# bluenote-1577/skani

Measured on NVIDIA H100. Metric: genome-pairs/sec, skani triangle 5k x 5 Mbp synthetic, higher is better.
Workload: dtype u64

## Files before the change

skani_b200/csrc/chain.cu:

```cuda
#include <cub/cub.cuh>

#include <algorithm>
#include <cmath>
#include <cstdlib>
#include <cstring>
#include <limits>
#include <numeric>

#include "chain_core.cuh"
#include "sk_internal.h"

namespace sk {

namespace tables {
#include "gbdt_tables.inc"
}

__constant__ unsigned char c_gbdt_feat[2][1365];
__constant__ float c_gbdt_thr[2][1365];
__constant__ float c_gbdt_leaf[2][1560];
__constant__ float c_gbdt_shrink[2];
__constant__ float c_gbdt_bias[2];

struct SetView {
// ... 1195 lines not shown
    feat[0][i] = tables::SK_GBDT_C125_FEAT[i]; feat[1][i] = tables::SK_GBDT_C200_FEAT[i];
    thr[0][i] = b2f(tables::SK_GBDT_C125_THR[i]); thr[1][i] = b2f(tables::SK_GBDT_C200_THR[i]);
  }
  for (int i = 0; i < 1560; i++) { leaf[0][i] = b2f(tables::SK_GBDT_C125_LEAF[i]); leaf[1][i] = b2f(tables::SK_GBDT_C200_LEAF[i]); }
  shrink[0] = b2f(SK_GBDT_C125_SHRINK_BITS); shrink[1] = b2f(SK_GBDT_C200_SHRINK_BITS);
  bias[0] = b2f(SK_GBDT_C125_BIAS_BITS); bias[1] = b2f(SK_GBDT_C200_BIAS_BITS);
  SK_CUDA(cudaMemcpyToSymbol(c_gbdt_feat, feat, sizeof(feat)));
  SK_CUDA(cudaMemcpyToSymbol(c_gbdt_thr, thr, sizeof(thr)));
  SK_CUDA(cudaMemcpyToSymbol(c_gbdt_leaf, leaf, sizeof(leaf)));
  SK_CUDA(cudaMemcpyToSymbol(c_gbdt_shrink, shrink, sizeof(shrink)));
  SK_CUDA(cudaMemcpyToSymbol(c_gbdt_bias, bias, sizeof(bias)));
  SK_CUDA(cudaDeviceSynchronize());
  if (ctx->device < 64) g_tables_uploaded[ctx->device] = true;
  return SK_OK;
}

static SetView view_of(const sk_sketch_set* s) {
  SetView v;
  v.pv_kmer = s->pv_kmer; v.pv_pos = s->pv_pos; v.pv_cc = s->pv_cc; v.pv_mult = s->pv_mult;
  v.kv_pos = s->kv_pos; v.kv_cc = s->kv_cc; v.ukmer = s->ukmer; v.ustart = s->ustart; v.ctg_rec_off = s->ctg_rec_off; v.ubucket = s->ubucket; v.htab = s->htab;
  return v;
}

static void build_meta(const sk_sketch_set* s, std::vector<GenomeMeta>& out) {
  out.resize(s->G);
  std::vector<uint32_t> tmp;
  for (uint32_t g = 0; g < s->G; g++) {
    GenomeMeta& m = out[g];
    m.seed_off = s->seed_off[g]; m.uk_off = s->uk_off[g]; m.ctg_off = s->ctg_off[g];
    m.n_rec = (uint32_t)(s->seed_off[g + 1] - s->seed_off[g]);
    m.n_uk = (uint32_t)(s->uk_off[g + 1] - s->uk_off[g]);
    m.n_ctg = (uint32_t)(s->ctg_off[g + 1] - s->ctg_off[g]);
    m.g = g; m.total_len = s->total_len[g]; m.pad = 0;
    m.ht_off = s->ht_off.empty() ? 0 : s->ht_off[g];
    m.ht_cap = s->ht_off.empty() ? 0 : (uint32_t)(s->ht_off[g + 1] - s->ht_off[g]);
    tmp.assign(s->ctg_len.begin() + s->ctg_off[g], s->ctg_len.begin() + s->ctg_off[g + 1]);
    uint64_t max_chunks = 0;
    for (uint32_t len : tmp) max_chunks += (len + (uint64_t)FRAGMENT_LENGTH - 1) / FRAGMENT_LENGTH;
    m.max_chunks = (uint32_t)std::min<uint64_t>(max_chunks, 0xFFFFFFFFu);
    std::sort(tmp.begin(), tmp.end());
    size_t n = tmp.size();
    m.q10 = n ? tmp[n * 10 / 100] : 0; m.q50 = n ? tmp[n * 50 / 100] : 0; m.q90 = n ? tmp[n * 90 / 100] : 0;
  }
}

static bool pair_switched(const sk_sketch_set* refs, uint32_t r, const sk_sketch_set* qs, uint32_t q, bool same_set) {
  auto mean_len = [](const sk_sketch_set* s, uint32_t g) {
    double sum = 0;
    for (uint64_t c = s->ctg_off[g]; c < s->ctg_off[g + 1]; c++) sum += (double)s->ctg_len[c];
    return sum / (double)(s->ctg_off[g + 1] - s->ctg_off[g]);
  };
  double mean_q = mean_len(qs, q), mean_r = mean_len(refs, r);
  double qp, rp;
  if (qs->total_len[q] > 100000 && refs->total_len[r] > 100000) {
    qp = (double)(qs->mk_off[q + 1] - qs->mk_off[q]) * (double)qs->sp.c;
    rp = (double)(refs->mk_off[r + 1] - refs->mk_off[r]) * (double)refs->sp.c;
  } else {
    qp = (double)qs->total_len[q]; rp = (double)refs->total_len[r];
  }
  double score_query = qp * std::min(mean_q, 300000.);
  double score_ref = rp * std::min(mean_r, 300000.);
  if (score_query == score_ref) {
    uint64_t rq = qs->name_rank[q] + ((same_set || qs->ranks_user_set) ? 0 : refs->G), rr = refs->name_rank[r];
    return rq > rr;
  }
  return score_query > score_ref;
}

struct BatchBuffers {
  std::vector<std::pair<void**, size_t>> reg;
};

template <typename T>
static int ensure(sk_ctx* ctx, T** p, size_t* cap, size_t need) {
  if (need <= *cap && *p) return SK_OK;
  if (*p) SK_CUDA(cudaFree(*p));
  *p = nullptr;
  size_t n = std::max<size_t>(need + need / 4, 1024);
  SK_CUDA(cudaMalloc((void**)p, n * sizeof(T)));
  *cap = n;
  return SK_OK;
}

struct ChainScratch {
  Workspace ws{};
  size_t cap_rec = 0, cap_pair = 0, cap_anc = 0, cap_chunk = 0, cap_iv = 0;
  size_t c_rec_nh = 0, c_rec_rs = 0, c_tile_off = 0;
  size_t c_stg_first = 0, c_stg_qctg = 0, c_stg_lo = 0, c_stg_hi = 0;
  size_t c_pairA = 0, c_pairC = 0, c_pairAbase = 0, c_pairCbase = 0, c_pairIbase = 0, c_pair_nint = 0, c_pair_sumlen = 0,
         c_pair_nchains = 0, c_pair_tqb = 0;
  size_t c_anc = 0, c_score = 0, c_ptr = 0, c_rootkey = 0, c_depth = 0;
  size_t c_chunk_size = 0, c_chunk_size_sorted = 0, c_chunk_id = 0, c_chunk_perm = 0, c_sort_tmp = 0;
  uint8_t* sort_tmp = nullptr;
  uint32_t* dbg_counts = nullptr; size_t c_dbg_counts = 0;
  size_t c_chunk_first = 0, c_chunk_pair = 0, c_chunk_qctg = 0, c_chunk_lo = 0, c_chunk_hi = 0, c_acc_total = 0, c_acc_rq0 = 0,
         c_acc_rq1 = 0, c_acc_tbcq = 0, c_acc_nint = 0, c_chunk_head = 0, c_chunk_est = 0, c_chunk_w = 0, c_chunk_valid = 0, c_chunk_nseeds = 0;
  size_t c_iv = 0, c_iv_keys = 0, c_iv_order = 0, c_iv_kept = 0, c_iv_next = 0, c_acc_list = 0, c_est_sorted = 0, c_w_sorted = 0;
  PairDesc* d_pairs = nullptr; size_t c_pairs = 0;
  sk_ani_result* d_out = nullptr; size_t c_out = 0;
  GenomeMeta *d_m0 = nullptr, *d_m1 = nullptr;
  size_t c_m0 = 0, c_m1 = 0;
  void free_all() {
    void* ptrs[] = {ws.chunk_size, ws.chunk_size_sorted, ws.chunk_id, ws.chunk_perm, sort_tmp, dbg_counts, ws.rec_nh, ws.rec_rs, ws.tile_off, ws.stg_first, ws.stg_qctg, ws.stg_lo, ws.stg_hi,
                    ws.pairA, ws.pairC, ws.pairAbase, ws.pairCbase, ws.pairIbase, ws.pair_nint, ws.pair_sumlen, ws.pair_nchains, ws.pair_tqb_ns, ws.anc,
                    ws.score, ws.ptr, ws.rootkey, ws.depth, ws.chunk_first, ws.chunk_pair, ws.chunk_qctg, ws.chunk_lo, ws.chunk_hi,
                    ws.acc_total, ws.acc_rq0, ws.acc_rq1, ws.acc_tbcq, ws.acc_nint, ws.chunk_head, ws.chunk_est, ws.chunk_w, ws.chunk_valid,
                    ws.chunk_nseeds, ws.iv, ws.iv_keys, ws.iv_order, ws.iv_kept, ws.iv_next, ws.acc_list, ws.est_sorted, ws.w_sorted, d_pairs, d_out, d_m0, d_m1};
    for (void* p : ptrs) if (p) cudaFree(p);
  }
};

struct HostPair { uint32_t ref, query; };

template <bool TAPS, int GL, int NE>
static int launch_dp_group(sk_ctx* ctx, uint32_t grid, uint64_t TC, const ChainParams& prm, const Workspace& ws, int dp_minb) {
  cudaStream_t st = ctx->stream;
  if (prm.band == GL * NE && dp_minb > 1) SK_LAUNCH(ctx, "dp_kernel", (dp_group_kernel<TAPS, GL, NE, true, 25><<<grid, 32, 0, st>>>(TC, prm, ws)));
  else if (prm.band == GL * NE) SK_LAUNCH(ctx, "dp_kernel", (dp_group_kernel<TAPS, GL, NE, true, 1><<<grid, 32, 0, st>>>(TC, prm, ws)));
  else SK_LAUNCH(ctx, "dp_kernel", (dp_group_kernel<TAPS, GL, NE, false, 1><<<grid, 32, 0, st>>>(TC, prm, ws)));
  return SK_OK;
}

static int launch_dp_select(sk_ctx* ctx, ChainScratch& S, uint32_t B, uint64_t TC, const ChainParams& prm, bool dp, bool taps) {
  cudaStream_t st = ctx->stream;
  Workspace& ws = S.ws;
  if (dp) {
    const uint32_t grid = (uint32_t)TC;
    const uint32_t nb = prm.band / 32 + 2;
#define DP_LAUNCH(NBV)                                                                                       \
  if (taps) SK_LAUNCH(ctx, "dp_kernel", (dp_warp_kernel<NBV, true><<<grid, 32, 0, st>>>(TC, prm, ws)));       \
  else SK_LAUNCH(ctx, "dp_kernel", (dp_warp_kernel<NBV, false><<<grid, 32, 0, st>>>(TC, prm, ws)));
    if (prm.band <= 24 && getenv("SK_DP_WARP") == nullptr) {
      const int dp_gl = getenv("SK_DP_GL") ? atoi(getenv("SK_DP_GL")) : 4;
      const int dp_minb = getenv("SK_DP_MINB") ? atoi(getenv("SK_DP_MINB")) : 25;
      const uint32_t gw = dp_gl == 4 ? 8 : 4;
      const uint32_t g4 = (uint32_t)((TC + gw - 1) / gw);
      SK_TRY(ensure(ctx, &ws.chunk_size, &S.c_chunk_size, TC)); SK_TRY(ensure(ctx, &ws.chunk_size_sorted, &S.c_chunk_size_sorted, TC));
      SK_TRY(ensure(ctx, &ws.chunk_id, &S.c_chunk_id, TC)); SK_TRY(ensure(ctx, &ws.chunk_perm, &S.c_chunk_perm, TC));
      chunk_size_kernel<<<(uint32_t)((TC + 255) / 256), 256, 0, st>>>(TC, ws); count_launch(ctx);
      size_t tb = 0;
      SK_CUDA(cub::DeviceRadixSort::SortPairsDescending(nullptr, tb, ws.chunk_size, ws.chunk_size_sorted, ws.chunk_id, ws.chunk_perm, (int)TC, 0, 32, st));
      SK_TRY(ensure(ctx, &S.sort_tmp, &S.c_sort_tmp, tb));
      SK_CUDA(cub::DeviceRadixSort::SortPairsDescending(S.sort_tmp, tb, ws.chunk_size, ws.chunk_size_sorted, ws.chunk_id, ws.chunk_perm, (int)TC, 0, 32, st));
#define DPG(GLV, NEV)                                                                                                   \
  {                                                                                                                    \
    if (taps) SK_TRY((launch_dp_group<true, GLV, NEV>(ctx, g4, TC, prm, ws, dp_minb)));                                \
    else SK_TRY((launch_dp_group<false, GLV, NEV>(ctx, g4, TC, prm, ws, dp_minb)));                                   \
  }
      if (dp_gl == 4) { if (prm.band <= 20) DPG(4, 5) else DPG(4, 6) }
      else { DPG(8, 3) }
#undef DPG
    } else if (nb <= 2) { DP_LAUNCH(2) } else if (nb <= 4) { DP_LAUNCH(4) } else if (nb <= 8) { DP_LAUNCH(8) }
    else if (nb <= 16) { DP_LAUNCH(16) } else { ctx->err = "c too small: chain band > 479 anchors is not supported"; return SK_ERR_PARAM; }
#undef DP_LAUNCH
  }
  SK_LAUNCH(ctx, "select_kernel", (select_kernel<<<B, CT, 0, st>>>(S.d_pairs, prm, ws)));
  return SK_OK;
}

static int copy_out_debug(sk_ctx* ctx, const Workspace& ws, const std::vector<PairDesc>& descs, size_t b0, uint32_t B,
                          const std::vector<uint64_t>& abase, const std::vector<uint64_t>& cbase, const std::vector<uint64_t>& ibase,
                          const uint32_t* dbg_counts, const sk_ani_result* host_out, sk_chain_debug* dbg) {
  const uint64_t TA = abase[B], TC = cbase[B], TI = ibase[B];
  std::vector<AnchorRec> anc(TA);
  std::vector<int32_t> score(TA);
  std::vector<uint32_t> ptr(TA), cq(TC), nseeds(TC), nint(B), w(TC), order(4 * TI);
  std::vector<uint64_t> cf(TC + 1);
  std::vector<IntervalKey> iv(TI);
  std::vector<uint8_t> kept(TI), valid(TC);
  std::vector<double> est(TC);
  std::vector<uint32_t> a_total(TC), a_rq0(TC), a_rq1(TC), a_tbcq(TC), a_nint(TC), counts(3 * TC);
  if (TA) {
    SK_CUDA(cudaMemcpy(anc.data(), ws.anc, TA * sizeof(AnchorRec), cudaMemcpyDeviceToHost));
    SK_CUDA(cudaMemcpy(score.data(), ws.score, TA * 4, cudaMemcpyDeviceToHost));
    SK_CUDA(cudaMemcpy(ptr.data(), ws.ptr, TA * 4, cudaMemcpyDeviceToHost));
  }
  if (TC) {
    SK_CUDA(cudaMemcpy(cf.data(), ws.chunk_first, (TC + 1) * 8, cudaMemcpyDeviceToHost));
    SK_CUDA(cudaMemcpy(cq.data(), ws.chunk_qctg, TC * 4, cudaMemcpyDeviceToHost));
    SK_CUDA(cudaMemcpy(nseeds.data(), ws.chunk_nseeds, TC * 4, cudaMemcpyDeviceToHost));
    SK_CUDA(cudaMemcpy(est.data(), ws.chunk_est, TC * 8, cudaMemcpyDeviceToHost));
    SK_CUDA(cudaMemcpy(w.data(), ws.chunk_w, TC * 4, cudaMemcpyDeviceToHost));
    SK_CUDA(cudaMemcpy(valid.data(), ws.chunk_valid, TC, cudaMemcpyDeviceToHost));
    SK_CUDA(cudaMemcpy(a_total.data(), ws.acc_total, TC * 4, cudaMemcpyDeviceToHost));
    SK_CUDA(cudaMemcpy(a_rq0.data(), ws.acc_rq0, TC * 4, cudaMemcpyDeviceToHost));
    SK_CUDA(cudaMemcpy(a_rq1.data(), ws.acc_rq1, TC * 4, cudaMemcpyDeviceToHost));
    SK_CUDA(cudaMemcpy(a_tbcq.data(), ws.acc_tbcq, TC * 4, cudaMemcpyDeviceToHost));
    SK_CUDA(cudaMemcpy(a_nint.data(), ws.acc_nint, TC * 4, cudaMemcpyDeviceToHost));
    SK_CUDA(cudaMemcpy(counts.data(), dbg_counts, TC * 12, cudaMemcpyDeviceToHost));
  }
  SK_CUDA(cudaMemcpy(nint.data(), ws.pair_nint, B * 4, cudaMemcpyDeviceToHost));
  if (TI) {
    SK_CUDA(cudaMemcpy(iv.data(), ws.iv, TI * sizeof(IntervalKey), cudaMemcpyDeviceToHost));
    SK_CUDA(cudaMemcpy(order.data(), ws.iv_order, 4 * TI * 4, cudaMemcpyDeviceToHost));
    SK_CUDA(cudaMemcpy(kept.data(), ws.iv_kept, TI, cudaMemcpyDeviceToHost));
  }
  for (uint32_t i = 0; i < B; i++) {
    sk_chain_debug* d = dbg + b0 + i;
    memset(d, 0, sizeof(*d));
    d->result = host_out[b0 + i];
    d->switched = descs[b0 + i].switched;
    const uint64_t a0 = abase[i], na = abase[i + 1] - a0, c0 = cbase[i], nc = cbase[i + 1] - c0, ib = ibase[i];
    const uint32_t ni = nint[i];
    if (ni > ibase[i + 1] - ib) { ctx->err = "chain debug: a pair has more intervals than its capacity"; return SK_ERR_STATE; }
    d->n_anchors = na; d->n_chunks = nc; d->n_intervals = ni;
    d->anchors = (uint32_t*)calloc(std::max<uint64_t>(na, 1), 20);
    d->score = (int64_t*)calloc(std::max<uint64_t>(na, 1), 8);
    d->pointer = (uint32_t*)calloc(std::max<uint64_t>(na, 1), 4);
    d->chunk_first = (uint32_t*)calloc(nc + 1, 4);
    d->chunk_nseeds = (uint32_t*)calloc(std::max<uint64_t>(nc, 1), 4);
    d->intervals = (int64_t*)calloc(std::max<uint32_t>(ni, 1), 11 * 8);
    d->chunk_stats = (uint32_t*)calloc(std::max<uint64_t>(nc, 1), 9 * 4);
    if (!d->anchors || !d->score || !d->pointer || !d->chunk_first || !d->chunk_nseeds || !d->intervals || !d->chunk_stats) {
      ctx->err = "chain debug: out of host memory"; return SK_ERR_STATE;
    }
    for (uint64_t c = 0; c < nc; c++) {
      const uint64_t x0 = cf[c0 + c] - a0, x1 = cf[c0 + c + 1] - a0;
      if (x0 > x1 || x1 > na) { ctx->err = "chain debug: chunk outside its pair's anchors"; return SK_ERR_STATE; }
      d->chunk_first[c] = (uint32_t)x0; d->chunk_nseeds[c] = nseeds[c0 + c];
      const uint64_t g = c0 + c;
      const uint32_t st[9] = {a_total[g], a_rq0[g], a_rq1[g], a_tbcq[g], a_nint[g], nseeds[g], counts[3 * g], counts[3 * g + 1],
                              counts[3 * g + 2]};
      memcpy(d->chunk_stats + 9 * c, st, sizeof(st));
      for (uint64_t x = x0; x < x1; x++) {
        const AnchorRec& a = anc[a0 + x];
        uint32_t* o = d->anchors + 5 * x;
        o[0] = cq[c0 + c]; o[1] = a.qpos; o[2] = a.rc >> 1; o[3] = a.rpos; o[4] = a.rc & 1u;
        d->score[x] = score[a0 + x]; d->pointer[x] = ptr[a0 + x];
      }
    }
    d->chunk_first[nc] = (uint32_t)na;
    uint32_t npow2 = 1;
    while (npow2 < ni) npow2 <<= 1;
    for (uint32_t j = 0; j < ni; j++) {
      const uint32_t oj = order[4 * ib + npow2 + j];
      if (oj >= ni) { ctx->err = "chain debug: interval order out of range"; return SK_ERR_STATE; }
      const IntervalKey& x = iv[ib + oj];
      int64_t* o = d->intervals + 11 * j;
      o[0] = iv_score(x); o[1] = iv_num_anchors(x); o[2] = iv_q0(x); o[3] = iv_q1(x); o[4] = iv_r0(x); o[5] = iv_r1(x);
      o[6] = iv_rctg(x); o[7] = iv_qctg(x); o[8] = iv_chunk(x); o[9] = iv_rev(x); o[10] = kept[ib + oj];
    }
    std::vector<std::pair<double, uint64_t>> es;
    for (uint64_t c = c0; c < c0 + nc; c++) if (valid[c]) es.push_back({est[c], w[c]});
    std::sort(es.begin(), es.end());
    d->n_ests = es.size();
    d->est = (double*)calloc(std::max<size_t>(es.size(), 1), 8);
    d->weight = (uint64_t*)calloc(std::max<size_t>(es.size(), 1), 8);
    if (!d->est || !d->weight) { ctx->err = "chain debug: out of host memory"; return SK_ERR_STATE; }
    for (size_t j = 0; j < es.size(); j++) { d->est[j] = es[j].first; d->weight[j] = es[j].second; }
  }
  return SK_OK;
}

static int run_batch(sk_ctx* ctx, ChainScratch& S, const sk_sketch_set* refs, const sk_sketch_set* qs, const std::vector<PairDesc>& descs,
                     size_t b0, size_t b1, uint64_t total_rec, uint64_t total_chunks, const std::vector<uint32_t>& tile_off, const ChainParams& prm, const SetView& v0, const SetView& v1,
                     sk_ani_result* host_out, sk_chain_debug* dbg) {
  cudaStream_t st = ctx->stream;
  const uint32_t B = (uint32_t)(b1 - b0);
  Workspace& ws = S.ws;
  const size_t NR = std::max<uint64_t>(total_rec, 1);
#define ENS(field, capf, n) SK_TRY(ensure(ctx, &ws.field, &S.capf, n))
  const size_t NS = std::max<uint64_t>(total_chunks, 1);
  ENS(rec_nh, c_rec_nh, NR); ENS(rec_rs, c_rec_rs, NR); ENS(tile_off, c_tile_off, B + 1);
  ENS(stg_first, c_stg_first, NS); ENS(stg_qctg, c_stg_qctg, NS); ENS(stg_lo, c_stg_lo, NS); ENS(stg_hi, c_stg_hi, NS);
  ENS(pairA, c_pairA, B); ENS(pairC, c_pairC, B); ENS(pairAbase, c_pairAbase, B + 1); ENS(pairCbase, c_pairCbase, B + 1);
  ENS(pairIbase, c_pairIbase, B + 1); ENS(pair_nint, c_pair_nint, B); ENS(pair_sumlen, c_pair_sumlen, B); ENS(pair_nchains, c_pair_nchains, B);
  ENS(pair_tqb_ns, c_pair_tqb, B);
  SK_TRY(ensure(ctx, &S.d_pairs, &S.c_pairs, B));
  SK_TRY(ensure(ctx, &S.d_out, &S.c_out, B));
  SK_CUDA(h2d_small(ctx, S.d_pairs, descs.data() + b0, B * sizeof(PairDesc)));
  SK_CUDA(cudaMemsetAsync(ws.pair_nint, 0, B * 4, st));
  SK_CUDA(cudaMemsetAsync(ws.pair_sumlen, 0, B * 4, st));
  SK_CUDA(cudaMemsetAsync(ws.pair_nchains, 0, B * 4, st));
  SK_CUDA(cudaMemsetAsync(ws.pair_tqb_ns, 0, B * 4, st));
  SK_CUDA(cudaMemsetAsync(ws.pairA, 0, B * 4, st));
  SK_CUDA(h2d_small(ctx, ws.tile_off, tile_off.data(), (B + 1) * 4));

  const uint32_t n_tiles = tile_off[B];
  if (n_tiles > 0) {
    size_t n_small = 0;
    for (size_t i = b0; i < b1; i++) {
      const PairDesc& d = descs[i];
      if (!d.valid) continue;
      const sk_sketch_set* rs_ = d.rset ? qs : refs;
      if (!rs_->ht_off.empty()) { const uint64_t cap = rs_->ht_off[d.rg + 1] - rs_->ht_off[d.rg]; if (cap && cap <= PROBE_STAGE_ENTRIES) n_small++; }
    }
    const bool staged = (getenv("SK_PROBE_TMA") ? atoi(getenv("SK_PROBE_TMA")) != 0 : true) && 2 * n_small >= (size_t)B;
    if (staged) SK_LAUNCH(ctx, "probe_kernel", (probe_kernel<true, PROBE_MINB><<<n_tiles, CT, 0, st>>>(S.d_pairs, B, v0, v1, S.d_m0, S.d_m1, prm, ws)));
    else SK_LAUNCH(ctx, "probe_kernel", (probe_kernel<false, PROBE_MINB><<<n_tiles, CT, 0, st>>>(S.d_pairs, B, v0, v1, S.d_m0, S.d_m1, prm, ws)));
  }
  std::vector<uint32_t> hA(B), hC(B);
  SK_CUDA(cudaMemcpyAsync(hA.data(), ws.pairA, B * 4, cudaMemcpyDeviceToHost, st));
  SK_CUDA(cudaStreamSynchronize(st));
  SK_CUDA(cudaGetLastError());
  std::vector<uint64_t> abase(B + 1, 0), cbase(B + 1, 0), ibase(B + 1, 0);
  for (uint32_t i = 0; i < B; i++) {
    abase[i + 1] = abase[i] + hA[i];
    ibase[i + 1] = ibase[i] + hA[i] / 3;
  }
  const uint64_t TA = abase[B], TI = ibase[B];
  SK_CUDA(h2d_small(ctx, ws.pairAbase, abase.data(), (B + 1) * 8));
  SK_CUDA(h2d_small(ctx, ws.pairIbase, ibase.data(), (B + 1) * 8));
  const size_t NA = std::max<uint64_t>(TA, 1), NI = std::max<uint64_t>(TI, 1);
  ENS(anc, c_anc, NA);
  SK_CUDA(cudaFuncSetAttribute(chunk_anchor_kernel<CHUNK_ANCHOR_MINB>, cudaFuncAttributeMaxDynamicSharedMemorySize,
                               (int)sizeof(ChunkAnchorSmem)));
  SK_LAUNCH(ctx, "chunk_anchor_kernel", (chunk_anchor_kernel<CHUNK_ANCHOR_MINB><<<B, CT, sizeof(ChunkAnchorSmem), st>>>(S.d_pairs, v0, v1, S.d_m0, S.d_m1, ws)));
  SK_CUDA(cudaMemcpyAsync(hC.data(), ws.pairC, B * 4, cudaMemcpyDeviceToHost, st));
  SK_CUDA(cudaStreamSynchronize(st));
  SK_CUDA(cudaGetLastError());
  for (uint32_t i = 0; i < B; i++) {
    if (hC[i] > descs[b0 + i].max_chunks) { ctx->err = "chain: a pair has more chunks than its contig-length bound"; return SK_ERR_STATE; }
    cbase[i + 1] = cbase[i] + hC[i];
  }
  const uint64_t TC = cbase[B];
  SK_CUDA(h2d_small(ctx, ws.pairCbase, cbase.data(), (B + 1) * 8));
  const size_t NCH = std::max<uint64_t>(TC, 1);
  ENS(score, c_score, dbg ? NA : 1); ENS(ptr, c_ptr, dbg ? NA : 1); ENS(rootkey, c_rootkey, NA); ENS(depth, c_depth, NA);
  ENS(chunk_first, c_chunk_first, NCH + 1); ENS(chunk_pair, c_chunk_pair, NCH); ENS(chunk_qctg, c_chunk_qctg, NCH);
  ENS(chunk_lo, c_chunk_lo, NCH); ENS(chunk_hi, c_chunk_hi, NCH); ENS(acc_total, c_acc_total, NCH); ENS(acc_rq0, c_acc_rq0, NCH);
  ENS(acc_rq1, c_acc_rq1, NCH); ENS(acc_tbcq, c_acc_tbcq, NCH); ENS(acc_nint, c_acc_nint, NCH); ENS(chunk_head, c_chunk_head, NCH);
  ENS(chunk_est, c_chunk_est, NCH); ENS(chunk_w, c_chunk_w, NCH); ENS(chunk_valid, c_chunk_valid, NCH); ENS(chunk_nseeds, c_chunk_nseeds, NCH);
  ENS(iv, c_iv, NI); ENS(iv_keys, c_iv_keys, 2 * NI + 8); ENS(iv_order, c_iv_order, 4 * NI + 8); ENS(iv_kept, c_iv_kept, NI); ENS(iv_next, c_iv_next, NI); ENS(acc_list, c_acc_list, NI);
  ENS(est_sorted, c_est_sorted, 4 * NCH + 8); ENS(w_sorted, c_w_sorted, 4 * NCH + 8);
#undef ENS
  if (dbg) SK_TRY(ensure(ctx, &S.dbg_counts, &S.c_dbg_counts, 3 * NCH));
  uint32_t* const dbg_counts = dbg ? S.dbg_counts : nullptr;
  if (TC > 0) {
    SK_CUDA(h2d_small(ctx, ws.chunk_first + TC, &TA, 8));
    SK_LAUNCH(ctx, "chunk_compact_kernel", (chunk_compact_kernel<<<B, CT, 0, st>>>(S.d_pairs, ws)));
    init_chunk_acc_kernel<<<(uint32_t)((TC + 255) / 256), 256, 0, st>>>(TC, ws); count_launch(ctx);
    SK_TRY(launch_dp_select(ctx, S, B, TC, prm, true, dbg != nullptr));
    SK_LAUNCH(ctx, "chunkstat_kernel", (chunkstat_kernel<<<(uint32_t)((TC + CS_WARPS * CS_PER_WARP - 1) / (CS_WARPS * CS_PER_WARP)), CS_WARPS * 32, 0, st>>>(TC, S.d_pairs, v0, v1, S.d_m0, S.d_m1, prm, ws, dbg_counts)));
  }
  const char* fr = getenv("SK_FINAL_FORCE_REDO");
  const int force_redo = (fr && atoi(fr) != 0) ? 1 : 0;
  SK_LAUNCH(ctx, "final_kernel", (final_kernel<<<B, FT, 0, st>>>(S.d_pairs, S.d_m0, S.d_m1, prm, ws, S.d_out, force_redo)));
  SK_CUDA(cudaMemcpyAsync(host_out + b0, S.d_out, B * sizeof(sk_ani_result), cudaMemcpyDeviceToHost, st));
  SK_CUDA(cudaStreamSynchronize(st));
  SK_CUDA(cudaGetLastError());

  if (dbg) SK_TRY(copy_out_debug(ctx, ws, descs, b0, B, abase, cbase, ibase, dbg_counts, host_out, dbg));
  return SK_OK;
}

static ChainScratch& chain_scratch(sk_ctx* ctx) {
  if (!ctx->chain_scratch) {
    ctx->chain_scratch = new ChainScratch();
    ctx->chain_scratch_free = [](void* p) { ((ChainScratch*)p)->free_all(); delete (ChainScratch*)p; };
  }
  return *(ChainScratch*)ctx->chain_scratch;
}

static int debug_dp_select(sk_ctx* ctx, uint32_t c, uint32_t k, const uint32_t* switched, const std::vector<uint64_t>& cbase,
                           const std::vector<uint64_t>& abase, const std::vector<uint64_t>& ibase, const std::vector<AnchorRec>& h_anc,
                           const std::vector<uint64_t>& h_first, const std::vector<uint32_t>& h_qctg,
                           const std::vector<IntervalKey>& h_iv, const std::vector<uint32_t>& h_nint, bool dp, sk_chain_debug* out,
                           uint32_t* pair_sums) {
  SK_CUDA(cudaSetDevice(ctx->device));
  cudaStream_t st = ctx->stream;
  const uint32_t B = (uint32_t)(cbase.size() - 1);
  ChainParams prm{};
  prm.c = c; prm.k = k; prm.band = BP_CHAIN_BAND / c; prm.model = -1;
  if (prm.band / 32 + 2 > 16) { ctx->err = "c too small: chain band > 479 anchors is not supported"; return SK_ERR_PARAM; }
  ChainScratch& S = chain_scratch(ctx);
  Workspace& ws = S.ws;
  const uint64_t TA = abase[B], TC = cbase[B], TI = ibase[B];
  const size_t NA = std::max<uint64_t>(TA, 1), NCH = std::max<uint64_t>(TC, 1), NI = std::max<uint64_t>(TI, 1);
#define ENS(field, capf, n) SK_TRY(ensure(ctx, &ws.field, &S.capf, n))
  ENS(pairCbase, c_pairCbase, B + 1); ENS(pairIbase, c_pairIbase, B + 1); ENS(pair_nint, c_pair_nint, B);
  ENS(pair_sumlen, c_pair_sumlen, B); ENS(pair_nchains, c_pair_nchains, B);
  ENS(anc, c_anc, NA); ENS(score, c_score, NA); ENS(ptr, c_ptr, NA); ENS(rootkey, c_rootkey, NA); ENS(depth, c_depth, NA);
  ENS(chunk_first, c_chunk_first, NCH + 1); ENS(chunk_pair, c_chunk_pair, NCH); ENS(chunk_qctg, c_chunk_qctg, NCH);
  ENS(acc_total, c_acc_total, NCH); ENS(acc_rq0, c_acc_rq0, NCH); ENS(acc_rq1, c_acc_rq1, NCH); ENS(acc_tbcq, c_acc_tbcq, NCH);
  ENS(acc_nint, c_acc_nint, NCH); ENS(chunk_head, c_chunk_head, NCH); ENS(chunk_est, c_chunk_est, NCH); ENS(chunk_w, c_chunk_w, NCH);
  ENS(chunk_valid, c_chunk_valid, NCH); ENS(chunk_nseeds, c_chunk_nseeds, NCH);
  ENS(iv, c_iv, NI); ENS(iv_keys, c_iv_keys, 2 * NI + 8); ENS(iv_order, c_iv_order, 4 * NI + 8); ENS(iv_kept, c_iv_kept, NI);
  ENS(iv_next, c_iv_next, NI); ENS(acc_list, c_acc_list, NI);
#undef ENS
  SK_TRY(ensure(ctx, &S.dbg_counts, &S.c_dbg_counts, 3 * NCH));
  SK_TRY(ensure(ctx, &S.d_pairs, &S.c_pairs, B));
  std::vector<PairDesc> descs(B);
  std::vector<uint32_t> h_pair(TC);
  for (uint32_t p = 0; p < B; p++) {
    PairDesc& d = descs[p];
    memset(&d, 0, sizeof(d));
    d.switched = switched[p] ? 1 : 0; d.valid = 1;
    for (uint64_t i = cbase[p]; i < cbase[p + 1]; i++) h_pair[i] = p;
  }
  SK_CUDA(cudaMemcpyAsync(S.d_pairs, descs.data(), B * sizeof(PairDesc), cudaMemcpyHostToDevice, st));
  SK_CUDA(cudaMemcpyAsync(ws.pairCbase, cbase.data(), (B + 1) * 8, cudaMemcpyHostToDevice, st));
  SK_CUDA(cudaMemcpyAsync(ws.pairIbase, ibase.data(), (B + 1) * 8, cudaMemcpyHostToDevice, st));
  SK_CUDA(cudaMemsetAsync(ws.pair_sumlen, 0, B * 4, st));
  SK_CUDA(cudaMemsetAsync(ws.pair_nchains, 0, B * 4, st));
  if (dp) SK_CUDA(cudaMemsetAsync(ws.pair_nint, 0, B * 4, st));
  else SK_CUDA(cudaMemcpyAsync(ws.pair_nint, h_nint.data(), B * 4, cudaMemcpyHostToDevice, st));
  if (TA) {
    SK_CUDA(cudaMemcpyAsync(ws.anc, h_anc.data(), TA * sizeof(AnchorRec), cudaMemcpyHostToDevice, st));
    SK_CUDA(cudaMemsetAsync(ws.score, 0, TA * 4, st));
    SK_CUDA(cudaMemsetAsync(ws.ptr, 0, TA * 4, st));
  }
  SK_CUDA(cudaMemcpyAsync(ws.chunk_first, h_first.data(), (TC + 1) * 8, cudaMemcpyHostToDevice, st));
  if (TC) {
    SK_CUDA(cudaMemcpyAsync(ws.chunk_pair, h_pair.data(), TC * 4, cudaMemcpyHostToDevice, st));
    SK_CUDA(cudaMemcpyAsync(ws.chunk_qctg, h_qctg.data(), TC * 4, cudaMemcpyHostToDevice, st));
    SK_CUDA(cudaMemsetAsync(ws.chunk_nseeds, 0, TC * 4, st));
    SK_CUDA(cudaMemsetAsync(ws.chunk_valid, 0, TC, st));
    SK_CUDA(cudaMemsetAsync(S.dbg_counts, 0, TC * 12, st));
  }
  if (TI && !dp) SK_CUDA(cudaMemcpyAsync(ws.iv, h_iv.data(), TI * sizeof(IntervalKey), cudaMemcpyHostToDevice, st));
  if (TC) {
    init_chunk_acc_kernel<<<(uint32_t)((TC + 255) / 256), 256, 0, st>>>(TC, ws); count_launch(ctx);
    SK_TRY(launch_dp_select(ctx, S, B, TC, prm, dp, true));
  }
  std::vector<sk_ani_result> res(B);
  memset(res.data(), 0, B * sizeof(sk_ani_result));
  std::vector<uint32_t> sl(B), nc(B);
  SK_CUDA(cudaMemcpyAsync(sl.data(), ws.pair_sumlen, B * 4, cudaMemcpyDeviceToHost, st));
  SK_CUDA(cudaMemcpyAsync(nc.data(), ws.pair_nchains, B * 4, cudaMemcpyDeviceToHost, st));
  SK_CUDA(cudaStreamSynchronize(st));
  SK_CUDA(cudaGetLastError());
  for (uint32_t p = 0; p < B; p++) { pair_sums[2 * p] = sl[p]; pair_sums[2 * p + 1] = nc[p]; }
  return copy_out_debug(ctx, ws, descs, 0, B, abase, cbase, ibase, S.dbg_counts, res.data(), out);
}

static int chain_impl(sk_ctx* ctx, const sk_sketch_set* refs, const sk_sketch_set* qs, const uint64_t* pairs, uint64_t n_pairs,
                      const sk_map_params* mp, sk_ani_result* out, sk_chain_debug* dbg) {
  SK_CUDA(cudaSetDevice(ctx->device));
  if (refs->sp.c != qs->sp.c || refs->sp.k != qs->sp.k) { ctx->err = "ref/query sketch parameters differ"; return SK_ERR_PARAM; }
  if (n_pairs == 0) return SK_OK;
  SK_TRY(upload_tables(ctx));
  ChainParams prm;
  prm.c = refs->sp.c; prm.k = refs->sp.k;
  prm.band = BP_CHAIN_BAND / refs->sp.c;
  prm.ushift = 2 * refs->sp.k > UBUCKET_BITS ? 2 * refs->sp.k - UBUCKET_BITS : 0;
  prm.robust = mp->robust; prm.median = mp->median;
  double fcc = mp->min_aligned_frac;
  if (fcc < 0.) fcc = 15.0 / 100.;
  prm.frac_cover_cutoff = fcc;
  prm.both_frac_cover_cutoff = mp->both_min_aligned_frac;
  prm.model = -1;
  if (mp->learned_ani) {
    long d125 = std::labs((long)refs->sp.c - 125), d200 = std::labs((long)refs->sp.c - 200);
    prm.model = d125 < d200 ? 0 : 1;
  }
  if (prm.band / 32 + 2 > 16) { ctx->err = "c too small: chain band > 479 anchors is not supported"; return SK_ERR_PARAM; }
  const bool same = (refs == qs);
  ChainScratch& S = chain_scratch(ctx);
  std::vector<GenomeMeta> m0, m1;
  build_meta(refs, m0);
  build_meta(qs, m1);
  SK_TRY(ensure(ctx, &S.d_m0, &S.c_m0, m0.size()));
  SK_TRY(ensure(ctx, &S.d_m1, &S.c_m1, m1.size()));
  SK_CUDA(h2d_small(ctx, S.d_m0, m0.data(), m0.size() * sizeof(GenomeMeta)));
  SK_CUDA(h2d_small(ctx, S.d_m1, m1.data(), m1.size() * sizeof(GenomeMeta)));
  const SetView v0 = view_of(refs), v1 = view_of(qs);
  std::vector<PairDesc> descs(n_pairs);
  for (uint64_t i = 0; i < n_pairs; i++) {
    uint32_t r = (uint32_t)(pairs[i] >> 32), q = (uint32_t)pairs[i];
    if (r >= refs->G || q >= qs->G) { ctx->err = "pair index out of range"; return SK_ERR_PARAM; }
    PairDesc& d = descs[i];
    d.ref_idx = r; d.query_idx = q; d.rec_off = 0; d.chunk_off = 0; d.max_chunks = 0; d.pad = 0;
    bool empty = (m0[r].n_ctg == 0 || m1[q].n_ctg == 0);
    d.valid = empty ? 0 : 1;
    bool sw = empty ? true : pair_switched(refs, r, qs, q, same);
    d.switched = sw ? 1 : 0;
    if (sw) { d.qset = 0; d.qg = r; d.rset = 1; d.rg = q; }
    else { d.qset = 1; d.qg = q; d.rset = 0; d.rg = r; }
  }
  const uint64_t REC_CAP = 128ull << 20;
  std::vector<uint32_t> tile_off;
  size_t b0 = 0;
  while (b0 < n_pairs) {
    size_t b1 = b0;
    uint64_t rec = 0, chunks = 0;
    tile_off.assign(1, 0);
    while (b1 < n_pairs && b1 - b0 < 65535) {
      PairDesc& d = descs[b1];
      const GenomeMeta* qm = d.valid ? &(d.qset ? m1 : m0)[d.qg] : nullptr;
      const uint64_t nr = qm ? qm->n_rec : 0;
      if (b1 > b0 && rec + nr > REC_CAP) break;
      d.rec_off = rec;
      d.chunk_off = chunks;
      d.max_chunks = qm ? qm->max_chunks : 0;
      rec += nr; chunks += d.max_chunks;
      tile_off.push_back(tile_off.back() + (uint32_t)((nr + TILE - 1) / TILE));
      b1++;
    }
    SK_TRY(run_batch(ctx, S, refs, qs, descs, b0, b1, rec, chunks, tile_off, prm, v0, v1, out, dbg));
    b0 = b1;
  }
  return SK_OK;
}

}

extern "C" {

int sk_chain_pairs(sk_ctx* ctx, const sk_sketch_set* refs, const sk_sketch_set* queries, const uint64_t* pairs, uint64_t n_pairs,
                   const sk_map_params* mp, sk_ani_result* out) {
  if (!ctx || !refs || !queries || !mp || (n_pairs && (!pairs || !out))) return SK_ERR_PARAM;
  return sk::chain_impl(ctx, refs, queries, pairs, n_pairs, mp, out, nullptr);
}

void sk_chain_debug_free(sk_chain_debug* d) {
  if (!d) return;
  free(d->anchors); free(d->chunk_first); free(d->chunk_nseeds); free(d->score); free(d->pointer); free(d->intervals);
  free(d->est); free(d->weight); free(d->chunk_stats);
  memset(d, 0, sizeof(*d));
}

int sk_debug_chunk_estimate(sk_ctx* ctx, uint64_t n, const uint32_t* inputs, uint32_t c, uint32_t k, double* est, uint32_t* weight,
                            uint32_t* valid) {
  if (!ctx || (n && (!inputs || !est || !weight || !valid)) || k == 0) return SK_ERR_PARAM;
  if (n == 0) return SK_OK;
  SK_CUDA(cudaSetDevice(ctx->device));
  cudaStream_t st = ctx->stream;
  uint32_t *d_in = nullptr, *d_w = nullptr, *d_v = nullptr;
  double* d_e = nullptr;
  int rc = SK_OK;
  cudaError_t e = cudaMalloc(&d_in, n * 32);
  if (e == cudaSuccess) e = cudaMalloc(&d_e, n * 8);
  if (e == cudaSuccess) e = cudaMalloc(&d_w, n * 4);
  if (e == cudaSuccess) e = cudaMalloc(&d_v, n * 4);
  if (e == cudaSuccess) e = cudaMemcpyAsync(d_in, inputs, n * 32, cudaMemcpyHostToDevice, st);
  if (e == cudaSuccess) {
    sk::debug_chunk_estimate_kernel<<<(uint32_t)((n + 255) / 256), 256, 0, st>>>(n, d_in, c, k, d_e, d_w, d_v);
    sk::count_launch(ctx);
    e = cudaGetLastError();
  }
  if (e == cudaSuccess) e = cudaMemcpyAsync(est, d_e, n * 8, cudaMemcpyDeviceToHost, st);
  if (e == cudaSuccess) e = cudaMemcpyAsync(weight, d_w, n * 4, cudaMemcpyDeviceToHost, st);
  if (e == cudaSuccess) e = cudaMemcpyAsync(valid, d_v, n * 4, cudaMemcpyDeviceToHost, st);
  if (e == cudaSuccess) e = cudaStreamSynchronize(st);
  if (e != cudaSuccess) { ctx->err = cudaGetErrorString(e); rc = SK_ERR_CUDA; }
  cudaFree(d_in); cudaFree(d_e); cudaFree(d_w); cudaFree(d_v);
  return rc;
}

int sk_debug_chain_anchors(sk_ctx* ctx, uint32_t c, uint32_t k, uint64_t n_pairs, const uint64_t* pair_chunk_off,
                           const uint64_t* chunk_anchor_off, const uint32_t* anchors, const uint32_t* switched, sk_chain_debug* out,
                           uint32_t* pair_sums) {
  if (!ctx || c == 0 || (n_pairs && (!pair_chunk_off || !chunk_anchor_off || !switched || !out || !pair_sums))) return SK_ERR_PARAM;
  if (n_pairs == 0) return SK_OK;
  if (n_pairs > 65535) { ctx->err = "debug chain: at most 65535 pairs"; return SK_ERR_PARAM; }
  memset(out, 0, n_pairs * sizeof(*out));
  const uint64_t TC = pair_chunk_off[n_pairs], TA = chunk_anchor_off[TC];
  if (pair_chunk_off[0] != 0 || chunk_anchor_off[0] != 0 || (TA && !anchors)) return SK_ERR_PARAM;
  std::vector<uint64_t> cbase(n_pairs + 1), abase(n_pairs + 1, 0), ibase(n_pairs + 1, 0), first(TC + 1);
  std::vector<uint32_t> qctg(TC);
  std::vector<sk::AnchorRec> anc(TA);
  for (uint64_t p = 0; p <= n_pairs; p++) {
    cbase[p] = pair_chunk_off[p];
    if (p && cbase[p] < cbase[p - 1]) { ctx->err = "debug chain: pair chunk offsets decrease"; return SK_ERR_PARAM; }
  }
  for (uint64_t p = 0; p < n_pairs; p++) {
    for (uint64_t ch = cbase[p]; ch < cbase[p + 1]; ch++) {
      const uint64_t a0 = chunk_anchor_off[ch], a1 = chunk_anchor_off[ch + 1];
      if (a1 <= a0) { ctx->err = "debug chain: every chunk holds at least one anchor"; return SK_ERR_PARAM; }
      first[ch] = a0;
      qctg[ch] = anchors[5 * a0];
      for (uint64_t i = a0; i < a1; i++) {
        const uint32_t* x = anchors + 5 * i;
        if (x[0] != qctg[ch]) { ctx->err = "debug chain: a chunk holds one query contig"; return SK_ERR_PARAM; }
        if (x[2] >= (1u << 30) || x[4] > 1u) { ctx->err = "debug chain: ref contig >= 2^30 or reverse flag > 1"; return SK_ERR_PARAM; }
        if (x[1] >= 0xFFFF0000u || x[3] >= 0xFFFF0000u) { ctx->err = "debug chain: position >= 2^32 - 65536"; return SK_ERR_PARAM; }
        if (i > a0) {
          const uint32_t* y = x - 5;
          const bool sorted = y[1] != x[1] ? y[1] < x[1] : y[2] != x[2] ? y[2] < x[2] : y[3] != x[3] ? y[3] < x[3] : y[4] <= x[4];
          if (!sorted) { ctx->err = "debug chain: the anchors of a chunk are not sorted by (qpos, rctg, rpos, rev)"; return SK_ERR_PARAM; }
        }
        anc[i].qpos = x[1]; anc[i].rpos = x[3]; anc[i].rc = (x[2] << 1) | x[4];
      }
// ... 66 lines not shown
```

Baseline: 46.28 million.

## Pipeline chain batches across two scratch slots with pinned host buffers and events

Splits the per-batch chain pipeline into probe/anchor/back/finish stages. Batches alternate between two scratch slots, so host-side prefix sums and launches for the next batch are interleaved with the current batch's GPU work. Stream synchronisations are replaced by event synchronisation on pinned host buffers, which also makes the device-to-host copies truly asynchronous. Everything still runs on a single stream, so overlap is limited to the host-side gaps. Duplicating the scratch doubles device memory use.

```diff
diff --git a/skani_b200/csrc/chain.cu b/skani_b200/csrc/chain.cu
--- a/skani_b200/csrc/chain.cu
+++ b/skani_b200/csrc/chain.cu
@@ -1301,7 +1301,18 @@
   return SK_OK;
 }
 
-struct ChainScratch {
+template <typename T>
+static int ensure_pinned(sk_ctx* ctx, T** p, size_t* cap, size_t need) {
+  if (need <= *cap && *p) return SK_OK;
+  if (*p) SK_CUDA(cudaFreeHost(*p));
+  *p = nullptr;
+  const size_t n = std::max<size_t>(need + need / 4, 1024);
+  SK_CUDA(cudaHostAlloc((void**)p, n * sizeof(T), cudaHostAllocDefault));
+  *cap = n;
+  return SK_OK;
+}
+
+struct BatchSlot {
   Workspace ws{};
   size_t cap_rec = 0, cap_pair = 0, cap_anc = 0, cap_chunk = 0, cap_iv = 0;
   size_t c_rec_nh = 0, c_rec_rs = 0, c_tile_off = 0;
@@ -1317,15 +1328,29 @@
   size_t c_iv = 0, c_iv_keys = 0, c_iv_order = 0, c_iv_kept = 0, c_iv_next = 0, c_acc_list = 0, c_est_sorted = 0, c_w_sorted = 0;
   PairDesc* d_pairs = nullptr; size_t c_pairs = 0;
   sk_ani_result* d_out = nullptr; size_t c_out = 0;
-  GenomeMeta *d_m0 = nullptr, *d_m1 = nullptr;
-  size_t c_m0 = 0, c_m1 = 0;
+  uint32_t *h_pairA = nullptr, *h_pairC = nullptr; sk_ani_result* h_out = nullptr;
+  size_t c_h_pairA = 0, c_h_pairC = 0, c_h_out = 0;
+  cudaEvent_t ev[3] = {nullptr, nullptr, nullptr};
   void free_all() {
     void* ptrs[] = {ws.chunk_size, ws.chunk_size_sorted, ws.chunk_id, ws.chunk_perm, sort_tmp, dbg_counts, ws.rec_nh, ws.rec_rs, ws.tile_off, ws.stg_first, ws.stg_qctg, ws.stg_lo, ws.stg_hi,
                     ws.pairA, ws.pairC, ws.pairAbase, ws.pairCbase, ws.pairIbase, ws.pair_nint, ws.pair_sumlen, ws.pair_nchains, ws.pair_tqb_ns, ws.anc,
                     ws.score, ws.ptr, ws.rootkey, ws.depth, ws.chunk_first, ws.chunk_pair, ws.chunk_qctg, ws.chunk_lo, ws.chunk_hi,
                     ws.acc_total, ws.acc_rq0, ws.acc_rq1, ws.acc_tbcq, ws.acc_nint, ws.chunk_head, ws.chunk_est, ws.chunk_w, ws.chunk_valid,
-                    ws.chunk_nseeds, ws.iv, ws.iv_keys, ws.iv_order, ws.iv_kept, ws.iv_next, ws.acc_list, ws.est_sorted, ws.w_sorted, d_pairs, d_out, d_m0, d_m1};
+                    ws.chunk_nseeds, ws.iv, ws.iv_keys, ws.iv_order, ws.iv_kept, ws.iv_next, ws.acc_list, ws.est_sorted, ws.w_sorted, d_pairs, d_out};
     for (void* p : ptrs) if (p) cudaFree(p);
+    for (void* p : {(void*)h_pairA, (void*)h_pairC, (void*)h_out}) if (p) cudaFreeHost(p);
+    for (cudaEvent_t e : ev) if (e) cudaEventDestroy(e);
+  }
+};
+
+struct ChainScratch {
+  BatchSlot slot[2];
+  GenomeMeta *d_m0 = nullptr, *d_m1 = nullptr;
+  size_t c_m0 = 0, c_m1 = 0;
+  void free_all() {
+    for (BatchSlot& s : slot) s.free_all();
+    if (d_m0) cudaFree(d_m0);
+    if (d_m1) cudaFree(d_m1);
   }
 };
 
@@ -1340,7 +1365,7 @@
   return SK_OK;
 }
 
-static int launch_dp_select(sk_ctx* ctx, ChainScratch& S, uint32_t B, uint64_t TC, const ChainParams& prm, bool dp, bool taps) {
+static int launch_dp_select(sk_ctx* ctx, BatchSlot& S, uint32_t B, uint64_t TC, const ChainParams& prm, bool dp, bool taps) {
   cudaStream_t st = ctx->stream;
   Workspace& ws = S.ws;
   if (dp) {
@@ -1471,12 +1496,36 @@
   return SK_OK;
 }
 
-static int run_batch(sk_ctx* ctx, ChainScratch& S, const sk_sketch_set* refs, const sk_sketch_set* qs, const std::vector<PairDesc>& descs,
-                     size_t b0, size_t b1, uint64_t total_rec, uint64_t total_chunks, const std::vector<uint32_t>& tile_off, const ChainParams& prm, const SetView& v0, const SetView& v1,
-                     sk_ani_result* host_out, sk_chain_debug* dbg) {
+struct BatchJob {
+  size_t b0 = 0, b1 = 0;
+  uint64_t rec = 0, chunks = 0;
+  std::vector<uint32_t> tile_off;
+  std::vector<uint64_t> abase, cbase, ibase;
+};
+
+struct ChainRun {
+  sk_ctx* ctx;
+  const sk_sketch_set *refs, *qs;
+  const std::vector<PairDesc>& descs;
+  const ChainParams& prm;
+  SetView v0, v1;
+  const GenomeMeta *d_m0, *d_m1;
+  sk_ani_result* host_out;
+  sk_chain_debug* dbg;
+  int probe(BatchJob& J, BatchSlot& S);
+  int anchor(BatchJob& J, BatchSlot& S);
+  int back(BatchJob& J, BatchSlot& S);
+  int finish(BatchJob& J, BatchSlot& S);
+};
+
+int ChainRun::probe(BatchJob& J, BatchSlot& S) {
   cudaStream_t st = ctx->stream;
+  const size_t b0 = J.b0, b1 = J.b1;
+  const std::vector<uint32_t>& tile_off = J.tile_off;
   const uint32_t B = (uint32_t)(b1 - b0);
   Workspace& ws = S.ws;
+  for (cudaEvent_t& e : S.ev) if (!e) SK_CUDA(cudaEventCreateWithFlags(&e, cudaEventDisableTiming));
+  const uint64_t total_rec = J.rec, total_chunks = J.chunks;
   const size_t NR = std::max<uint64_t>(total_rec, 1);
 #define ENS(field, capf, n) SK_TRY(ensure(ctx, &ws.field, &S.capf, n))
   const size_t NS = std::max<uint64_t>(total_chunks, 1);
@@ -1485,8 +1534,11 @@
   ENS(pairA, c_pairA, B); ENS(pairC, c_pairC, B); ENS(pairAbase, c_pairAbase, B + 1); ENS(pairCbase, c_pairCbase, B + 1);
   ENS(pairIbase, c_pairIbase, B + 1); ENS(pair_nint, c_pair_nint, B); ENS(pair_sumlen, c_pair_sumlen, B); ENS(pair_nchains, c_pair_nchains, B);
   ENS(pair_tqb_ns, c_pair_tqb, B);
+#undef ENS
   SK_TRY(ensure(ctx, &S.d_pairs, &S.c_pairs, B));
   SK_TRY(ensure(ctx, &S.d_out, &S.c_out, B));
+  SK_TRY(ensure_pinned(ctx, &S.h_pairA, &S.c_h_pairA, B)); SK_TRY(ensure_pinned(ctx, &S.h_pairC, &S.c_h_pairC, B));
+  SK_TRY(ensure_pinned(ctx, &S.h_out, &S.c_h_out, B));
   SK_CUDA(h2d_small(ctx, S.d_pairs, descs.data() + b0, B * sizeof(PairDesc)));
   SK_CUDA(cudaMemsetAsync(ws.pair_nint, 0, B * 4, st));
   SK_CUDA(cudaMemsetAsync(ws.pair_sumlen, 0, B * 4, st));
@@ -1505,36 +1557,56 @@
       if (!rs_->ht_off.empty()) { const uint64_t cap = rs_->ht_off[d.rg + 1] - rs_->ht_off[d.rg]; if (cap && cap <= PROBE_STAGE_ENTRIES) n_small++; }
     }
     const bool staged = (getenv("SK_PROBE_TMA") ? atoi(getenv("SK_PROBE_TMA")) != 0 : true) && 2 * n_small >= (size_t)B;
-    if (staged) SK_LAUNCH(ctx, "probe_kernel", (probe_kernel<true, PROBE_MINB><<<n_tiles, CT, 0, st>>>(S.d_pairs, B, v0, v1, S.d_m0, S.d_m1, prm, ws)));
-    else SK_LAUNCH(ctx, "probe_kernel", (probe_kernel<false, PROBE_MINB><<<n_tiles, CT, 0, st>>>(S.d_pairs, B, v0, v1, S.d_m0, S.d_m1, prm, ws)));
-  }
-  std::vector<uint32_t> hA(B), hC(B);
-  SK_CUDA(cudaMemcpyAsync(hA.data(), ws.pairA, B * 4, cudaMemcpyDeviceToHost, st));
-  SK_CUDA(cudaStreamSynchronize(st));
+    if (staged) SK_LAUNCH(ctx, "probe_kernel", (probe_kernel<true, PROBE_MINB><<<n_tiles, CT, 0, st>>>(S.d_pairs, B, v0, v1, d_m0, d_m1, prm, ws)));
+    else SK_LAUNCH(ctx, "probe_kernel", (probe_kernel<false, PROBE_MINB><<<n_tiles, CT, 0, st>>>(S.d_pairs, B, v0, v1, d_m0, d_m1, prm, ws)));
+  }
+  SK_CUDA(cudaMemcpyAsync(S.h_pairA, ws.pairA, B * 4, cudaMemcpyDeviceToHost, st));
+  SK_CUDA(cudaEventRecord(S.ev[0], st));
+  return SK_OK;
+}
+
+int ChainRun::anchor(BatchJob& J, BatchSlot& S) {
+  cudaStream_t st = ctx->stream;
+  const uint32_t B = (uint32_t)(J.b1 - J.b0);
+  Workspace& ws = S.ws;
+  SK_CUDA(cudaEventSynchronize(S.ev[0]));
   SK_CUDA(cudaGetLastError());
-  std::vector<uint64_t> abase(B + 1, 0), cbase(B + 1, 0), ibase(B + 1, 0);
+  const uint32_t* hA = S.h_pairA;
+  std::vector<uint64_t>&abase = J.abase, &ibase = J.ibase;
+  abase.assign(B + 1, 0); ibase.assign(B + 1, 0);
   for (uint32_t i = 0; i < B; i++) {
     abase[i + 1] = abase[i] + hA[i];
     ibase[i + 1] = ibase[i] + hA[i] / 3;
   }
-  const uint64_t TA = abase[B], TI = ibase[B];
   SK_CUDA(h2d_small(ctx, ws.pairAbase, abase.data(), (B + 1) * 8));
   SK_CUDA(h2d_small(ctx, ws.pairIbase, ibase.data(), (B + 1) * 8));
-  const size_t NA = std::max<uint64_t>(TA, 1), NI = std::max<uint64_t>(TI, 1);
-  ENS(anc, c_anc, NA);
+  SK_TRY(ensure(ctx, &ws.anc, &S.c_anc, std::max<uint64_t>(abase[B], 1)));
   SK_CUDA(cudaFuncSetAttribute(chunk_anchor_kernel<CHUNK_ANCHOR_MINB>, cudaFuncAttributeMaxDynamicSharedMemorySize,
                                (int)sizeof(ChunkAnchorSmem)));
-  SK_LAUNCH(ctx, "chunk_anchor_kernel", (chunk_anchor_kernel<CHUNK_ANCHOR_MINB><<<B, CT, sizeof(ChunkAnchorSmem), st>>>(S.d_pairs, v0, v1, S.d_m0, S.d_m1, ws)));
-  SK_CUDA(cudaMemcpyAsync(hC.data(), ws.pairC, B * 4, cudaMemcpyDeviceToHost, st));
-  SK_CUDA(cudaStreamSynchronize(st));
+  SK_LAUNCH(ctx, "chunk_anchor_kernel", (chunk_anchor_kernel<CHUNK_ANCHOR_MINB><<<B, CT, sizeof(ChunkAnchorSmem), st>>>(S.d_pairs, v0, v1, d_m0, d_m1, ws)));
+  SK_CUDA(cudaMemcpyAsync(S.h_pairC, ws.pairC, B * 4, cudaMemcpyDeviceToHost, st));
+  SK_CUDA(cudaEventRecord(S.ev[1], st));
+  return SK_OK;
+}
+
+int ChainRun::back(BatchJob& J, BatchSlot& S) {
+  cudaStream_t st = ctx->stream;
+  const size_t b0 = J.b0;
+  const uint32_t B = (uint32_t)(J.b1 - b0);
+  Workspace& ws = S.ws;
+  SK_CUDA(cudaEventSynchronize(S.ev[1]));
   SK_CUDA(cudaGetLastError());
+  const uint32_t* hC = S.h_pairC;
+  std::vector<uint64_t>& cbase = J.cbase;
+  cbase.assign(B + 1, 0);
   for (uint32_t i = 0; i < B; i++) {
     if (hC[i] > descs[b0 + i].max_chunks) { ctx->err = "chain: a pair has more chunks than its contig-length bound"; return SK_ERR_STATE; }
     cbase[i + 1] = cbase[i] + hC[i];
   }
-  const uint64_t TC = cbase[B];
+  const uint64_t TA = J.abase[B], TI = J.ibase[B], TC = cbase[B];
   SK_CUDA(h2d_small(ctx, ws.pairCbase, cbase.data(), (B + 1) * 8));
-  const size_t NCH = std::max<uint64_t>(TC, 1);
+  const size_t NA = std::max<uint64_t>(TA, 1), NI = std::max<uint64_t>(TI, 1), NCH = std::max<uint64_t>(TC, 1);
+#define ENS(field, capf, n) SK_TRY(ensure(ctx, &ws.field, &S.capf, n))
   ENS(score, c_score, dbg ? NA : 1); ENS(ptr, c_ptr, dbg ? NA : 1); ENS(rootkey, c_rootkey, NA); ENS(depth, c_depth, NA);
   ENS(chunk_first, c_chunk_first, NCH + 1); ENS(chunk_pair, c_chunk_pair, NCH); ENS(chunk_qctg, c_chunk_qctg, NCH);
   ENS(chunk_lo, c_chunk_lo, NCH); ENS(chunk_hi, c_chunk_hi, NCH); ENS(acc_total, c_acc_total, NCH); ENS(acc_rq0, c_acc_rq0, NCH);
@@ -1550,16 +1622,22 @@
     SK_LAUNCH(ctx, "chunk_compact_kernel", (chunk_compact_kernel<<<B, CT, 0, st>>>(S.d_pairs, ws)));
     init_chunk_acc_kernel<<<(uint32_t)((TC + 255) / 256), 256, 0, st>>>(TC, ws); count_launch(ctx);
     SK_TRY(launch_dp_select(ctx, S, B, TC, prm, true, dbg != nullptr));
-    SK_LAUNCH(ctx, "chunkstat_kernel", (chunkstat_kernel<<<(uint32_t)((TC + CS_WARPS * CS_PER_WARP - 1) / (CS_WARPS * CS_PER_WARP)), CS_WARPS * 32, 0, st>>>(TC, S.d_pairs, v0, v1, S.d_m0, S.d_m1, prm, ws, dbg_counts)));
+    SK_LAUNCH(ctx, "chunkstat_kernel", (chunkstat_kernel<<<(uint32_t)((TC + CS_WARPS * CS_PER_WARP - 1) / (CS_WARPS * CS_PER_WARP)), CS_WARPS * 32, 0, st>>>(TC, S.d_pairs, v0, v1, d_m0, d_m1, prm, ws, dbg_counts)));
   }
   const char* fr = getenv("SK_FINAL_FORCE_REDO");
   const int force_redo = (fr && atoi(fr) != 0) ? 1 : 0;
-  SK_LAUNCH(ctx, "final_kernel", (final_kernel<<<B, FT, 0, st>>>(S.d_pairs, S.d_m0, S.d_m1, prm, ws, S.d_out, force_redo)));
-  SK_CUDA(cudaMemcpyAsync(host_out + b0, S.d_out, B * sizeof(sk_ani_result), cudaMemcpyDeviceToHost, st));
-  SK_CUDA(cudaStreamSynchronize(st));
+  SK_LAUNCH(ctx, "final_kernel", (final_kernel<<<B, FT, 0, st>>>(S.d_pairs, d_m0, d_m1, prm, ws, S.d_out, force_redo)));
+  SK_CUDA(cudaMemcpyAsync(S.h_out, S.d_out, B * sizeof(sk_ani_result), cudaMemcpyDeviceToHost, st));
+  SK_CUDA(cudaEventRecord(S.ev[2], st));
+  return SK_OK;
+}
+
+int ChainRun::finish(BatchJob& J, BatchSlot& S) {
+  const uint32_t B = (uint32_t)(J.b1 - J.b0);
+  SK_CUDA(cudaEventSynchronize(S.ev[2]));
   SK_CUDA(cudaGetLastError());
-
-  if (dbg) SK_TRY(copy_out_debug(ctx, ws, descs, b0, B, abase, cbase, ibase, dbg_counts, host_out, dbg));
+  memcpy(host_out + J.b0, S.h_out, B * sizeof(sk_ani_result));
+  if (dbg) SK_TRY(copy_out_debug(ctx, S.ws, descs, J.b0, B, J.abase, J.cbase, J.ibase, S.dbg_counts, host_out, dbg));
   return SK_OK;
 }
 
@@ -1582,7 +1660,7 @@
   ChainParams prm{};
   prm.c = c; prm.k = k; prm.band = BP_CHAIN_BAND / c; prm.model = -1;
   if (prm.band / 32 + 2 > 16) { ctx->err = "c too small: chain band > 479 anchors is not supported"; return SK_ERR_PARAM; }
-  ChainScratch& S = chain_scratch(ctx);
+  BatchSlot& S = chain_scratch(ctx).slot[0];
   Workspace& ws = S.ws;
   const uint64_t TA = abase[B], TC = cbase[B], TI = ibase[B];
   const size_t NA = std::max<uint64_t>(TA, 1), NCH = std::max<uint64_t>(TC, 1), NI = std::max<uint64_t>(TI, 1);
@@ -1687,13 +1765,15 @@
     if (sw) { d.qset = 0; d.qg = r; d.rset = 1; d.rg = q; }
     else { d.qset = 1; d.qg = q; d.rset = 0; d.rg = r; }
   }
-  const uint64_t REC_CAP = 128ull << 20;
-  std::vector<uint32_t> tile_off;
+  const char* cap_env = getenv("SK_CHAIN_BATCH_RECORDS");
+  const uint64_t REC_CAP = cap_env ? std::max<uint64_t>(1, strtoull(cap_env, nullptr, 10)) : 128ull << 20;
+  std::vector<BatchJob> jobs;
   size_t b0 = 0;
   while (b0 < n_pairs) {
+    BatchJob J;
     size_t b1 = b0;
     uint64_t rec = 0, chunks = 0;
-    tile_off.assign(1, 0);
+    J.tile_off.assign(1, 0);
     while (b1 < n_pairs && b1 - b0 < 65535) {
       PairDesc& d = descs[b1];
       const GenomeMeta* qm = d.valid ? &(d.qset ? m1 : m0)[d.qg] : nullptr;
@@ -1703,11 +1783,31 @@
       d.chunk_off = chunks;
       d.max_chunks = qm ? qm->max_chunks : 0;
       rec += nr; chunks += d.max_chunks;
-      tile_off.push_back(tile_off.back() + (uint32_t)((nr + TILE - 1) / TILE));
+      J.tile_off.push_back(J.tile_off.back() + (uint32_t)((nr + TILE - 1) / TILE));
       b1++;
     }
-    SK_TRY(run_batch(ctx, S, refs, qs, descs, b0, b1, rec, chunks, tile_off, prm, v0, v1, out, dbg));
+    J.b0 = b0; J.b1 = b1; J.rec = rec; J.chunks = chunks;
+    jobs.push_back(std::move(J));
     b0 = b1;
+  }
+  ChainRun run{ctx, refs, qs, descs, prm, v0, v1, S.d_m0, S.d_m1, out, dbg};
+  const size_t n = jobs.size();
+  if (dbg) {
+    for (BatchJob& J : jobs) {
+      BatchSlot& s0 = S.slot[0];
+      SK_TRY(run.probe(J, s0)); SK_TRY(run.anchor(J, s0)); SK_TRY(run.back(J, s0)); SK_TRY(run.finish(J, s0));
+    }
+    return SK_OK;
+  }
+  SK_TRY(run.probe(jobs[0], S.slot[0]));
+  SK_TRY(run.anchor(jobs[0], S.slot[0]));
+  for (size_t i = 0; i < n; i++) {
+    BatchSlot& si = S.slot[i & 1];
+    BatchSlot& sn = S.slot[(i + 1) & 1];
+    if (i + 1 < n) SK_TRY(run.probe(jobs[i + 1], sn));
+    SK_TRY(run.back(jobs[i], si));
+    if (i + 1 < n) SK_TRY(run.anchor(jobs[i + 1], sn));
+    SK_TRY(run.finish(jobs[i], si));
   }
   return SK_OK;
 }
```

Result: faster. 47.46 million, median of 6 (+2.5%).
